# angela000/DQNFlappyBird

Hardware: AMD Instinct MI355X
Metric: env steps/sec (whole node) + DQN grad-steps/sec, 80x80x4 batch=32 (higher is better)
Workload: dtype f32

## Files before the change

### dqnflappybird_amd/csrc/fb_common.h

```cpp
#pragma once
#include <hip/hip_runtime.h>
#include <stdarg.h>
#include <stdint.h>
#include <stdio.h>
#include <string.h>
#include "../../include/fbdqn.h"

extern thread_local char fb_err_buf[512];
int fb_set_error(int code, const char *fmt, ...);

#define FB_CHECK_HIP(expr)                                                                     \
    do {                                                                                       \
        hipError_t e_ = (expr);                                                                \
        if (e_ != hipSuccess)                                                                  \
            return fb_set_error(FB_ERR_HIP, "%s failed: %s (%s:%d)", #expr, hipGetErrorString(e_), \
                                __FILE__, __LINE__);                                           \
    } while (0)

#define FB_REQUIRE(cond, ...)                                          \
    do {                                                               \
        if (!(cond)) return fb_set_error(FB_ERR_INVALID, __VA_ARGS__); \
    } while (0)

#define FB_LAUNCH_CHECK() FB_CHECK_HIP(hipGetLastError())
// ... 32 lines not shown
#define FB_STREAM_SAMPLE 2u
#define FB_STREAM_PER 3u
#define FB_STREAM_INIT 4u
#define FB_STREAM_EVAL 5u

struct fb_u4 { uint32_t x, y, z, w; };

__host__ __device__ static inline fb_u4 fb_philox(uint32_t k0, uint32_t k1, uint32_t c0, uint32_t c1,
                                                  uint32_t c2, uint32_t c3) {
#pragma unroll
    for (int r = 0; r < 10; r++) {
        uint64_t p0 = (uint64_t)0xD2511F53u * c0, p1 = (uint64_t)0xCD9E8D57u * c2;
        uint32_t n0 = (uint32_t)(p1 >> 32) ^ c1 ^ k0, n1 = (uint32_t)p1;
        uint32_t n2 = (uint32_t)(p0 >> 32) ^ c3 ^ k1, n3 = (uint32_t)p0;
        c0 = n0; c1 = n1; c2 = n2; c3 = n3;
        k0 += 0x9E3779B9u; k1 += 0xBB67AE85u;
    }
    return fb_u4{c0, c1, c2, c3};
}

struct FbMT { uint32_t mt[624]; uint32_t idx; };

struct FbSplitFlags;
struct FbSampleCtx { FbMT *mt; int *error; long long n; FbSplitFlags *gate; unsigned long long gate_val; long long newest_from; int wait_last_round; };
struct FbSampleRider { FbSampleCtx ctx; int k; long long setsize; long long *out; };
struct NetOff { int bf1, wv, bv, wq, bq, n; };
struct HeadCore {
    const float *hf; int stot, nks; float *q; int FC, A, dueling; NetOff off;
    uint8_t *actions; float epsilon; uint32_t seed_lo, seed_hi, step_lo, step_hi;
};
struct FbHeadRider { HeadCore c; const float *params; int on; unsigned long long *on_arrival; unsigned long long arrival_val; };
struct FbEvalRider {
    const int32_t *env_of;
    int32_t *ep_k, *ep_len;
    int32_t *score, *length; uint8_t *trunc;
    int episodes;
    unsigned *live;
    unsigned long long *done_step;
    unsigned long long step;
};
struct FbGatherCtx {
    long long cap; int n_envs, t_f, kind;
    const unsigned long long *bits; const uint8_t *act; const float *rew; const uint8_t *term; int *error;
    int nstep; double gamma;
};
struct FbGatherRider { FbGatherCtx c; long long steps; int B; const long long *idx; uint8_t *s, *s2, *a; float *r; uint8_t *t; };
int fb_replay_gather_rider(fb_replay_t h, int batch, const int64_t *idx, uint8_t *s, uint8_t *s2, uint8_t *a, float *r, uint8_t *t,
                           FbGatherRider *rider);
struct FbRingSrc { FbGatherCtx c; long long steps; const long long *idx; uint8_t *a; float *r; uint8_t *t; };
int fb_replay_ring_src(fb_replay_t h, int batch, const int64_t *idx, uint8_t *a, float *r, uint8_t *t, FbRingSrc *out);
int fb_qnet_train_step_ring(fb_qnet_t h, int algo, int batch, const FbRingSrc *ring, const float *isw, double gamma, float *loss,
                            float *abs_err, float *flat_grad, void *stream, const FbSampleRider *rider = nullptr, const struct FbSplitCtx *split = nullptr);
struct FbSplitFlags {
    unsigned long long c_entry, p0[7];
    unsigned long long trunk_done, p2[7];
    unsigned long long fc1_done, p3[7];
    unsigned long long env_done, p4[7];
    unsigned long long last_round, p8[7];
    unsigned clean_count;
    unsigned timeouts[7];
};
struct FbSplitCtx {
    hipStream_t tstream;
    FbSplitFlags *f;
    unsigned long long seq;
    const void *probed_stream; int probed_ok;
};
int fb_split_probe(FbSplitCtx *ctx, void *stream);
int fb_streams_concurrent(hipStream_t side, hipStream_t caller);
hipStream_t fb_side_stream_beside(hipStream_t caller, int priority, hipStream_t current, int *ok);
FbSplitCtx *fb_qnet_split_ctx(fb_qnet_t h);
int fb_replay_sample_gated(fb_replay_t h, int batch, int64_t *idx, const FbSplitCtx *ctx, void *stream, int wait_last_round = 0);
int fb_split_wait(const FbSplitCtx *ctx, const unsigned long long *flag, unsigned long long v, void *stream);
int fb_split_set(const FbSplitCtx *ctx, unsigned long long *flag, unsigned long long v, void *stream);
int fb_qnet_refresh_planes(fb_qnet_t h, void *stream);
int fb_qnet_profile_ring(fb_qnet_t h, int kernel, int reps, int algo, int batch, const FbRingSrc *ring, float *loss, void *stream);
struct FbPushRider { unsigned long long *bits; uint8_t *act; float *rew; uint8_t *term; long long *steps_dev; long long steps_new; };
int fb_env_step_rider(fb_env_t h, const uint8_t *actions, uint8_t *frames, uint64_t *frame_bits, float *reward, uint8_t *terminal,
                      int32_t *score, const FbSampleRider *rider, const FbPushRider *push, const FbHeadRider *head, void *stream);
int fb_qnet_num_actions(fb_qnet_t h);
int fb_qnet_is_c51(fb_qnet_t h);
int fb_qnet_c51_eval_head(fb_qnet_t h, const FbHeadRider *hd, int n, const int32_t *key_of, void *stream);
int fb_qnet_eval_trunk(fb_qnet_t h, const uint8_t *nib_states, int n, FbHeadRider *head, void *stream);
int fb_qnet_max_rows(fb_qnet_t h);
hipStream_t fb_qnet_side_stream(fb_qnet_t h);
void *fb_qnet_get_grad_event(fb_qnet_t h);
void *fb_qnet_take_grad_event_recorded(fb_qnet_t h);
int fb_qnet_check_step(fb_qnet_t h, int n_envs, int train_batch);
int fb_env_num_envs(fb_env_t h);
int fb_replay_num_envs(fb_replay_t h);
int fb_replay_is_prioritized(fb_replay_t h);
int fb_replay_check_gamma(fb_replay_t h, double gamma, const char *who);
int fb_replay_check_complete(fb_replay_t h, int pushes_ahead, const char *who);
double fb_replay_bootstrap_gamma(fb_replay_t h, double gamma);
int fb_replay_update_priorities_keep(fb_replay_t h, int batch, const int64_t *idx, const float *abs_err, void *stream);
// ... 16 lines not shown
```

### dqnflappybird_amd/csrc/fb_common.hip

```cpp
#include <execinfo.h>
#include <fcntl.h>
#include <signal.h>
#include <stdlib.h>
#include <unistd.h>
#include "fb_common.h"

thread_local char fb_err_buf[512] = "";

int fb_set_error(int code, const char *fmt, ...) {
    va_list ap;
    va_start(ap, fmt);
    vsnprintf(fb_err_buf, sizeof(fb_err_buf), fmt, ap);
    va_end(ap);
    return code;
}

extern "C" const char *fb_last_error(void) { return fb_err_buf; }

static struct sigaction fb_prev_abrt;
static bool fb_abrt_installed = false;
static int fb_abrt_log_fd = -1;
static void fb_abort_backtrace(int sig, siginfo_t *info, void *ctx) {
    static const char msg[] = "\n[libfbdqn] SIGABRT: native stack of the aborting thread\n";
    void *frames[64];
// ... 153 lines not shown
        if (hipStreamSynchronize(S) != hipSuccess || hipStreamSynchronize(C) != hipSuccess) return 0;
        unsigned long long st[3];
        if (hipMemcpy(st, &W->first, sizeof(st), hipMemcpyDeviceToHost) != hipSuccess) return 0;
        if (st[1] <= st[0]) return 0;
        const double frac = st[2] <= st[0] ? 0.0 : (double)(st[2] - st[0]) / (double)(st[1] - st[0]);
        if (frac < best) best = frac;
    }
    double worst_ratio = 1e9, alone_us = 0, beside_us = 0;
    for (int trial = 0; trial < 3 && worst_ratio >= 1.0; trial++) {
        unsigned long long st[5];
        const unsigned long long init[5] = {~0ull, 0ull, 0ull, ~0ull, 0ull};
        if (hipMemcpy(&W->first, init, sizeof(init), hipMemcpyHostToDevice) != hipSuccess) return 0;
        for (int i = 0; i < 8; i++) hipLaunchKernelGGL(probe_hold_kernel, dim3(1), dim3(64), 0, C, &W->first, &W->last, 50LL);
        if (hipStreamSynchronize(C) != hipSuccess || hipMemcpy(st, &W->first, sizeof(st), hipMemcpyDeviceToHost) != hipSuccess || st[1] <= st[0]) return 0;
        const double alone = (double)(st[1] - st[0]) / 100.0;
        if (hipMemcpy(&W->first, init, sizeof(init), hipMemcpyHostToDevice) != hipSuccess) return 0;
        hipLaunchKernelGGL(probe_hold_kernel, dim3(1), dim3(64), 0, S, &W->first2, &W->last2, 8000LL);
        for (int i = 0; i < 8; i++) hipLaunchKernelGGL(probe_hold_kernel, dim3(1), dim3(64), 0, C, &W->first, &W->last, 50LL);
        if (hipStreamSynchronize(S) != hipSuccess || hipStreamSynchronize(C) != hipSuccess) return 0;
        if (hipMemcpy(st, &W->first, sizeof(st), hipMemcpyDeviceToHost) != hipSuccess || st[1] <= st[0]) return 0;
        const double beside = (double)(st[1] - st[0]) / 100.0, ratio = beside / (2.0 * alone + 10.0);
        if (ratio < worst_ratio) { worst_ratio = ratio; alone_us = alone; beside_us = beside; }
    }
    if (getenv("FB_SIDE_PROBE_DEBUG"))
        fprintf(stderr, "[fb] side stream %p beside %p: a launch on it started %.2f of the way through a long launch on the caller's; eight small launches on the caller's took %.1f us beside "
                        "a long workgroup on it, %.1f alone\n", (void *)S, (void *)C, best, beside_us, alone_us);
    return best < 0.5 && worst_ratio < 1.0;
}

hipStream_t fb_side_stream_beside(hipStream_t C, int priority, hipStream_t current, int *ok) {
    bool good = current && fb_streams_concurrent(current, C);
    for (int attempt = 0; !good && attempt < 6; attempt++) {
        hipStream_t ts = nullptr;
        if (hipStreamCreateWithPriority(&ts, hipStreamNonBlocking, priority) != hipSuccess) break;
        if (current) { (void)hipStreamSynchronize(current); (void)hipStreamDestroy(current); }
        current = ts;
        good = fb_streams_concurrent(current, C);
    }
    (void)hipGetLastError();
    if (ok) *ok = good ? 1 : 0;
    return current;
}

static int fb_vec_split_flag = -1;
static bool fb_vec_split_enabled() {
    if (fb_vec_split_flag < 0) fb_vec_split_flag = !(getenv("FB_VEC_SPLIT") && atoi(getenv("FB_VEC_SPLIT")) == 0);
    return fb_vec_split_flag != 0;
}
extern "C" int fb_vec_step_set_schedule(int split) { fb_vec_split_flag = split ? 1 : 0; return FB_OK; }

// ... 8 lines not shown
        FB_REQUIRE(is_c51_algo(algo) == (fb_qnet_is_c51(net) != 0),
                   "%s: a C51 net takes a C51 algo (FB_ALGO_C51, _DOUBLE, _PER, _DOUBLE_PER), and those algos take a C51 net only (algo %d)", "fb_vec_step", algo);
        if (!is_per_algo(algo))
            FB_REQUIRE(!fb_replay_is_prioritized(replay), "%s: C51 trains from a uniform memory only (prioritized replay with C51 is not supported)", "fb_vec_step");
    }
    FB_REQUIRE(per == (fb_replay_is_prioritized(replay) != 0), "fb_vec_step: algo %d and the memory's kind (uniform / prioritized) do not match", algo);
    FB_REQUIRE(n_envs == fb_env_num_envs(env) && n_envs == fb_replay_num_envs(replay), "fb_vec_step: n_envs %d does not match the env (%d) / replay (%d) handles",
               n_envs, fb_env_num_envs(env), fb_replay_num_envs(replay));
    if (train) FB_REQUIRE(b->idx && b->s && b->s2 && b->a && b->r && b->t && b->loss, "fb_vec_step: NULL training buffer");
    {
        const int rc0 = fb_qnet_check_step(net, n_envs, train ? batch : -1);
        if (rc0 != FB_OK) return rc0;
        const int rc1 = fb_replay_check_gamma(replay, gamma, "fb_vec_step");
        if (rc1 != FB_OK) return rc1;
        const int rc2 = train ? fb_replay_check_complete(replay, 1, "fb_vec_step") : FB_OK;
        if (rc2 != FB_OK) return rc2;
    }
    gamma = fb_replay_bootstrap_gamma(replay, gamma);
    if (fb_vec_split_enabled() && train && !per && n_envs >= 256 && batch < 256 && fb_env_can_carry_head(env) && fb_qnet_num_actions(net) == 2 &&
        !fb_qnet_is_c51(net)) {
        hipStream_t A = fb_stream(stream);
        hipStreamCaptureStatus cap = hipStreamCaptureStatusNone;
        (void)hipStreamIsCapturing(A, &cap);
        FbSampleRider probe;
        FbSplitCtx *sc = cap == hipStreamCaptureStatusNone && fb_replay_sample_rider(replay, batch, b->idx, &probe) ? fb_qnet_split_ctx(net) : nullptr;
        if (sc && !fb_split_probe(sc, stream)) sc = nullptr;
        if (sc) {
            hipStream_t C = A, S = sc->tstream;
            FbSplitFlags *F = sc->f;
            sc->seq += 1;
            static const bool last_round_on = !(getenv("FB_SPLIT_LAST_ROUND") && atoi(getenv("FB_SPLIT_LAST_ROUND")) == 0);
            const int trunk_wgs = (n_envs + 4) / 5, wait_last_round = last_round_on && n_envs >= 4096 && trunk_wgs % 256 != 0;
            if (!fb_replay_sample_gated(replay, batch, b->idx, sc, C, wait_last_round)) { sc->seq -= 1; return fb_set_error(FB_ERR_HIP, "fb_vec_step: the gated draw could not be launched"); }
            int rc = fb_split_wait(sc, &F->c_entry, sc->seq, S);
            FbHeadRider hrider;
            if (rc == FB_OK) rc = fb_qnet_act_nib_rider(net, b->nib, n_envs, epsilon, seed, step, b->actions, &hrider, S, sc);
            if (rc != FB_OK) { (void)hipStreamSynchronize(S); return rc; }
            hrider.on_arrival = &F->fc1_done; hrider.arrival_val = sc->seq;
            FbPushRider prider;
            fb_replay_begin_push_rider(replay, &prider);
            FbRingSrc ring;
            rc = fb_replay_ring_src(replay, batch, b->idx, b->a, b->r, b->t, &ring);
            if (rc == FB_OK) rc = fb_qnet_train_step_ring(net, algo, batch, &ring, nullptr, gamma, b->loss, nullptr, b->flat_grad, C, nullptr, sc);
            const int rc2 = fb_env_step_rider(env, b->actions, nullptr, b->frame_bits, b->reward, b->terminal, b->score, nullptr, &prider, &hrider, S);
            const int rc3 = fb_split_set(sc, &F->env_done, sc->seq, S);
            return rc != FB_OK ? rc : rc2 != FB_OK ? rc2 : rc3;
        }
    }
    static const bool store_ahead = !(getenv("FB_PER_STORE_AHEAD") && atoi(getenv("FB_PER_STORE_AHEAD")) == 0);
    int sampled = 0;
    if (per && store_ahead && fb_replay_per_store_ahead(replay, stream) && train)
        sampled = fb_replay_sample_ahead(replay, batch, b->idx, b->isw, b->isw32, stream);
    FbHeadRider hrider;
    static const bool head_rides = !(getenv("FB_VEC_HEAD_RIDER") && atoi(getenv("FB_VEC_HEAD_RIDER")) == 0);
    const int have_h = head_rides && fb_env_can_carry_head(env) && fb_qnet_num_actions(net) == 2 && !fb_qnet_is_c51(net);
    int rc = have_h ? fb_qnet_act_nib_rider(net, b->nib, n_envs, epsilon, seed, step, b->actions, &hrider, stream)
                    : fb_qnet_act_nib(net, b->nib, n_envs, epsilon, seed, step, b->actions, nullptr, stream);
    if (rc != FB_OK) return rc;
    FbSampleRider srider;
    FbPushRider prider;
    static const bool sample_rides = !(getenv("FB_VEC_SAMPLE_RIDER") && atoi(getenv("FB_VEC_SAMPLE_RIDER")) == 0);
    const int have_s = train && sample_rides ? fb_replay_sample_rider(replay, batch, b->idx, &srider) : 0;
    const int have_p = fb_replay_begin_push_rider(replay, &prider);
    rc = fb_env_step_rider(env, b->actions, nullptr, b->frame_bits, b->reward, b->terminal, b->score, have_s ? &srider : nullptr,
                           have_p ? &prider : nullptr, have_h ? &hrider : nullptr, stream);
    if (rc != FB_OK) return rc;
// ... 74 lines not shown
```

### dqnflappybird_amd/csrc/fb_qnet.hip

```cpp
#include <math.h>
#include <stdlib.h>
#include "fb_common.h"

#ifndef FK_ABL
#define FK_ABL 0
#endif
#ifndef BW_ABL
#define BW_ABL 0
#endif

namespace {

typedef float f32x16 __attribute__((ext_vector_type(16)));

constexpr int OFF_W1 = 0, OFF_B1 = 8192, OFF_W2 = 8224, OFF_B2 = 40992, OFF_W3 = 41056, OFF_B3 = 77920,
              OFF_WF1 = 77984;
constexpr int CONV_PARAMS = OFF_WF1;
#include "fb_head.h"
#include "fb_sampler.h"
#include "fb_gather.h"
constexpr int MAXTB = 256;


struct Slice { const float *params; const uint8_t *states; int s_off, count; const uint16_t *w1s; int fshift; };
// ... 3080 lines not shown
    return FB_OK;
}

__global__ void flag_wait_kernel(const unsigned long long *flag, unsigned long long v, unsigned *timeouts) { if (threadIdx.x == 0) fb_flag_wait(flag, v, timeouts); }
__global__ void flag_set_kernel(unsigned long long *flag, unsigned long long v) { fb_flag_store(flag, v); }

FbSplitCtx *fb_qnet_split_ctx(fb_qnet_t h) {
    if (!h) return nullptr;
    if (h->split) return h->split->tstream ? h->split : nullptr;
    FbSplitCtx *c = new FbSplitCtx();
    memset(c, 0, sizeof(*c));
    h->split = c;
    int lo = 0, hi = 0;
    bool ok = hipMalloc((void **)&c->f, sizeof(FbSplitFlags)) == hipSuccess && hipMemset(c->f, 0, sizeof(FbSplitFlags)) == hipSuccess;
    hipStream_t ts = nullptr;
    ok = ok && hipDeviceGetStreamPriorityRange(&lo, &hi) == hipSuccess && hipStreamCreateWithPriority(&ts, hipStreamNonBlocking, lo) == hipSuccess;
    if (!ok) { (void)hipGetLastError(); return nullptr; }
    c->tstream = ts;
    return c;
}

int fb_split_probe(FbSplitCtx *c, void *stream) {
    if (!c || !c->tstream) return 0;
    if (c->probed_stream == stream && c->seq > 0) return c->probed_ok;
    int lo = 0, hi = 0, ok = 0;
    if (hipDeviceGetStreamPriorityRange(&lo, &hi) != hipSuccess) return 0;
    c->tstream = fb_side_stream_beside(reinterpret_cast<hipStream_t>(stream), lo, c->tstream, &ok);
    c->probed_stream = stream; c->probed_ok = ok;
    return ok;
}

int fb_split_wait(const FbSplitCtx *c, const unsigned long long *flag, unsigned long long v, void *stream) {
    hipLaunchKernelGGL(flag_wait_kernel, dim3(1), dim3(64), 0, fb_stream(stream), flag, v, &c->f->timeouts[1]);
    FB_LAUNCH_CHECK();
    return FB_OK;
}

int fb_split_set(const FbSplitCtx *, unsigned long long *flag, unsigned long long v, void *stream) {
    hipLaunchKernelGGL(flag_set_kernel, dim3(1), dim3(1), 0, fb_stream(stream), flag, v);
    FB_LAUNCH_CHECK();
    return FB_OK;
}

extern "C" int fb_qnet_split_stats(fb_qnet_t h, int64_t *steps_host, int64_t *clean_host) {
    FB_REQUIRE(h && steps_host && clean_host, "fb_qnet_split_stats: NULL argument");
    *steps_host = 0; *clean_host = 0;
    if (!h->split || !h->split->tstream) return FB_OK;
    FB_CHECK_HIP(hipDeviceSynchronize());
    unsigned v[8] = {0};
    FB_CHECK_HIP(hipMemcpy(v, &h->split->f->clean_count, sizeof(v), hipMemcpyDeviceToHost));
    FB_REQUIRE(!(v[1] | v[2] | v[3] | v[4] | v[5] | v[6]), "fb_qnet_split_stats: waits between the two chains of the split schedule gave up after 1 s (the draw %u, the side stream's entry %u, "
// ... 729 lines not shown
```

### dqnflappybird_amd/csrc/fb_replay.hip

```cpp
#include <math.h>
#include "fb_common.h"

namespace {

constexpr int WORDS = 100;
constexpr int MAXB = 256;
constexpr int MAXH = 23;

struct ReplayDev {
    long long steps;
    long long per_pointer, per_size;
    double beta;
    unsigned int done_ctr;
    unsigned int philox_calls;
    int error;
};

struct ReplayParams {
    long long cap;
    int n_envs, t_f, kind;
    unsigned long long *bits;
    uint8_t *act; float *rew; uint8_t *term;
    ReplayDev *dev;
    double *tree, *maxt, *mint;
// ... 65 lines not shown
template <bool CURRENT>
__global__ __launch_bounds__(256) void gather_kernel(ReplayParams P, long long steps, int B, const long long *__restrict__ idx,
                                                     uint4 *__restrict__ s, uint4 *__restrict__ s2,
                                                     uint8_t *__restrict__ a, float *__restrict__ r,
                                                     uint8_t *__restrict__ t) {
    gather_body<CURRENT>(gather_ctx(P), steps, B, idx, s, s2, a, r, t, (long long)blockIdx.x * 256 + threadIdx.x);
}

__device__ __forceinline__ FbSampleCtx sample_ctx(const ReplayParams &P, long long steps) {
    return FbSampleCtx{P.mt, &P.dev->error, population(P, steps)};
}

__global__ __launch_bounds__(64) void sample_cpython_kernel(ReplayParams P, int k, long long setsize,
                                                            long long *__restrict__ out) {
    __shared__ uint32_t mt[624];
    __shared__ int pool[FB_SAMPLE_POOL + FB_SAMPLE_TAB];
    sample_cpython_body(sample_ctx(P, P.dev->steps), k, setsize, out, mt, pool);
}

__global__ __launch_bounds__(64) void sample_gated_kernel(FbSampleRider r) {
    __shared__ uint32_t mt[624];
    __shared__ int pool[FB_SAMPLE_POOL + FB_SAMPLE_TAB];
    sample_cpython_body(r.ctx, r.k, r.setsize, r.out, mt, pool);
}

__global__ __launch_bounds__(64) void push_sample_kernel(ReplayParams P, long long steps, const uint8_t *__restrict__ frames,
                                                         const unsigned long long *__restrict__ fbits,
                                                         const uint8_t *__restrict__ a, const float *__restrict__ r,
                                                         const uint8_t *__restrict__ t, int k, long long setsize,
                                                         long long *__restrict__ out) {
    __shared__ uint32_t mt[624];
    __shared__ int pool[FB_SAMPLE_POOL + FB_SAMPLE_TAB];
    if (blockIdx.x == gridDim.x - 1) { sample_cpython_body(sample_ctx(P, steps + 1), k, setsize, out, mt, pool); return; }
    const int lane = threadIdx.x;
    for (int e = blockIdx.x; e < P.n_envs; e += gridDim.x - 1) {
        unsigned long long *dst = P.bits + frame_off(P, steps + 1, e);
        if (fbits) {
            for (int w = lane; w < WORDS; w += 64) dst[w] = fbits[(size_t)e * WORDS + w];
        } else {
            for (int w = 0; w < WORDS; w++) {
                const unsigned long long m = __ballot(frames[(size_t)e * 6400 + w * 64 + lane] != 0);
                if (lane == 0) dst[w] = m;
            }
        }
        if (lane == 0) {
            const size_t mo = (size_t)(steps % P.t_f) * P.n_envs + e;
// ... 462 lines not shown
        for (;;) {
            const long long cl = 2 * parent + 1;
            if (cl >= len) break;
            const double left = P.tree[cl];
            if (v <= left) parent = cl;
            else { v -= left; parent = cl + 1; }
        }
        const double prob = P.tree[parent] / total;
        const double min_prob = P.mint[0] / total;
        idx_out[tid] = parent;
        const double wgt = pow(prob / min_prob, -beta);
        isw_out[tid] = wgt;
        if (isw32_out) isw32_out[tid] = (float)wgt;
    }
    if (tid == 0) { P.dev->beta = beta; P.dev->philox_calls = call + 1; }
}

}

struct fb_replay {
    ReplayParams P;
    FbMT *h_mt;
    long long host_steps;
    int per_mode;
    hipStream_t side;
    hipEvent_t ev_fork, ev_store, ev_upd;
    bool store_ahead;
    bool upd_pending;
    bool store_forked;
    const void *side_for; bool side_checked; int side_ok; int side_prio;
};

static bool per_side_usable(fb_replay *h, void *stream) {
    if (!h->side) return false;
    if (h->side_checked && h->side_for == stream) return h->side_ok != 0;
    if (h->store_ahead || h->upd_pending) return h->side_checked && h->side_ok != 0;
    h->side = fb_side_stream_beside(fb_stream(stream), h->side_prio, h->side, &h->side_ok);
    h->side_for = stream; h->side_checked = true;
    return h->side_ok != 0;
}


static int per_join(fb_replay *h, hipStream_t st) {
    if (h->upd_pending) {
        FB_CHECK_HIP(hipStreamWaitEvent(st, h->ev_upd, 0));
        h->upd_pending = false;
    }
    return FB_OK;
}

static int replay_create(int64_t capacity, int n_envs, int kind, int ring_n, fb_replay_t *out) {
    fb_replay *h = new fb_replay();
    memset(h, 0, sizeof(*h));
    ReplayParams &P = h->P;
    P.cap = capacity; P.n_envs = n_envs; P.kind = kind;
    P.nstep = 1; P.gamma = 0.0;
    P.t_f = (int)((capacity + n_envs - 1) / n_envs) + ring_n + 5;
    const size_t slots = (size_t)P.t_f * n_envs;
    hipError_t e = hipMalloc(&P.bits, slots * WORDS * sizeof(unsigned long long));
    if (e == hipSuccess) e = hipMemset(P.bits, 0, slots * WORDS * sizeof(unsigned long long));
    if (e == hipSuccess) e = hipMalloc(&P.act, slots);
    if (e == hipSuccess) e = hipMemset(P.act, 0, slots);
    if (e == hipSuccess) e = hipMalloc(&P.rew, slots * sizeof(float));
    if (e == hipSuccess) e = hipMemset(P.rew, 0, slots * sizeof(float));
    if (e == hipSuccess) e = hipMalloc(&P.term, slots);
    if (e == hipSuccess) e = hipMemset(P.term, 0, slots);
    if (e == hipSuccess) e = hipMalloc(&P.dev, sizeof(ReplayDev));
    if (e == hipSuccess) e = hipMemset(P.dev, 0, sizeof(ReplayDev));
    if (e == hipSuccess) e = hipMalloc(&P.mt, sizeof(FbMT));
    if (e == hipSuccess && kind == FB_REPLAY_PER) {
        const size_t nb = sizeof(double) * (size_t)(2 * capacity - 1);
        e = hipMalloc(&P.tree, nb);
        if (e == hipSuccess) e = hipMalloc(&P.maxt, nb);
        if (e == hipSuccess) e = hipMalloc(&P.mint, nb);
    }
    if (e != hipSuccess) {
        fb_set_error(e == hipErrorOutOfMemory ? FB_ERR_NOMEM : FB_ERR_HIP, "fb_replay_create: %s", hipGetErrorString(e));
        fb_replay_destroy(h);
        return e == hipErrorOutOfMemory ? FB_ERR_NOMEM : FB_ERR_HIP;
    }
    if (kind == FB_REPLAY_PER) {
        int prio_lo = 0, prio_hi = 0;
        (void)hipDeviceGetStreamPriorityRange(&prio_lo, &prio_hi);
        h->side_prio = prio_hi;
        if (hipStreamCreateWithPriority(&h->side, hipStreamNonBlocking, h->side_prio) != hipSuccess ||
            hipEventCreateWithFlags(&h->ev_fork, hipEventDisableTiming) != hipSuccess ||
            hipEventCreateWithFlags(&h->ev_store, hipEventDisableTiming) != hipSuccess ||
            hipEventCreateWithFlags(&h->ev_upd, hipEventDisableTiming) != hipSuccess) {
            fb_set_error(FB_ERR_HIP, "fb_replay_create: stream / event creation failed");
            fb_replay_destroy(h);
            return FB_ERR_HIP;
        }
// ... 10 lines not shown
    FB_REQUIRE(n_envs >= 1 && n_envs <= (1 << 22), "fb_replay_create: n_envs out of range");
    FB_REQUIRE(kind == FB_REPLAY_UNIFORM || kind == FB_REPLAY_PER, "fb_replay_create: kind must be 0 or 1");
    return replay_create(capacity, n_envs, kind, 1, out);
}

extern "C" int fb_replay_create_nstep(int64_t capacity, int n_envs, int kind, int n, double gamma, fb_replay_t *out) {
    FB_REQUIRE(out, "fb_replay_create_nstep: out is NULL");
    FB_REQUIRE(capacity >= 1 && capacity < (1ll << 22), "fb_replay_create_nstep: capacity %lld out of range", (long long)capacity);
    FB_REQUIRE(n_envs >= 1 && n_envs <= (1 << 22), "fb_replay_create_nstep: n_envs out of range");
    FB_REQUIRE(kind == FB_REPLAY_UNIFORM || kind == FB_REPLAY_PER, "fb_replay_create_nstep: kind must be 0 or 1");
    FB_REQUIRE(n >= 1 && n <= FB_NSTEP_MAX, "fb_replay_create_nstep: n = %d is outside 1..%d", n, FB_NSTEP_MAX);
    FB_REQUIRE(capacity >= (long long)n * n_envs, "fb_replay_create_nstep: capacity %lld < n x n_envs = %lld", (long long)capacity,
               (long long)n * n_envs);
    const int rc = replay_create(capacity, n_envs, kind, kind == FB_REPLAY_PER ? n : 1, out);
    if (rc != FB_OK) return rc;
    (*out)->P.nstep = n;
    (*out)->P.gamma = n > 1 ? gamma : 0.0;
    return FB_OK;
}

extern "C" int fb_replay_destroy(fb_replay_t h) {
    if (!h) return FB_OK;
    ReplayParams &P = h->P;
    void *ptrs[] = {P.bits, P.act, P.rew, P.term, P.dev, P.mt, P.tree, P.maxt, P.mint};
    for (void *p : ptrs) if (p) (void)hipFree(p);
    if (h->side) { (void)hipStreamSynchronize(h->side); (void)hipStreamDestroy(h->side); }
    if (h->ev_fork) (void)hipEventDestroy(h->ev_fork);
    if (h->ev_store) (void)hipEventDestroy(h->ev_store);
    if (h->ev_upd) (void)hipEventDestroy(h->ev_upd);
    delete h;
    return FB_OK;
}

extern "C" int fb_replay_seed(fb_replay_t h, int rng_kind, uint64_t seed) {
    FB_REQUIRE(h, "fb_replay_seed: NULL handle");
    FB_REQUIRE(rng_kind >= 0 && rng_kind <= 2, "fb_replay_seed: rng_kind must be 0 (cpython), 1 (philox) or 2 (numpy)");
    FbMT s;
    if (rng_kind == FB_RNG_NUMPY) fb_mt_init_genrand_host(&s, (uint32_t)seed);
    else {
        uint32_t key[2] = {(uint32_t)seed, (uint32_t)(seed >> 32)};
        fb_mt_init_by_array_host(&s, key, key[1] ? 2 : 1);
    }
    FB_CHECK_HIP(hipDeviceSynchronize());
    FB_CHECK_HIP(hipMemcpy(h->P.mt, &s, sizeof(FbMT), hipMemcpyHostToDevice));
    h->P.rng_kind = rng_kind;
    h->P.seed_lo = (uint32_t)seed; h->P.seed_hi = (uint32_t)(seed >> 32);
    return FB_OK;
}

extern "C" int fb_replay_reset(fb_replay_t h, const uint8_t *frames, const uint64_t *frame_bits, void *stream) {
    FB_REQUIRE(h, "fb_replay_reset: NULL handle");
    h->host_steps = 0;
    ReplayParams &P = h->P;
    hipStream_t st = fb_stream(stream);
    if (P.kind == FB_REPLAY_PER) {
        if (h->side) {
            FB_CHECK_HIP(hipStreamSynchronize(h->side));
            h->store_ahead = false; h->upd_pending = false;
        }
        const long long nn = 2 * P.cap - 1;
        FB_CHECK_HIP(hipMemsetAsync(P.tree, 0, sizeof(double) * nn, st));
        FB_CHECK_HIP(hipMemsetAsync(P.maxt, 0, sizeof(double) * nn, st));
        hipLaunchKernelGGL(fill_f64_kernel, dim3(256), dim3(256), 0, st, P.mint, nn, (double)INFINITY);
        FB_LAUNCH_CHECK();
    }
    if (!frames && !frame_bits) {
        FB_CHECK_HIP(hipMemsetAsync(P.bits, 0, (size_t)P.n_envs * WORDS * sizeof(unsigned long long), st));
        FB_CHECK_HIP(hipMemsetAsync(P.dev, 0, sizeof(ReplayDev), st));
        ReplayDev d; memset(&d, 0, sizeof(d)); d.beta = 0.4;
        FB_CHECK_HIP(hipStreamSynchronize(st));
        FB_CHECK_HIP(hipMemcpy(P.dev, &d, sizeof(d), hipMemcpyHostToDevice));
        return FB_OK;
    }
    hipLaunchKernelGGL(reset_kernel, dim3(P.n_envs), dim3(64), 0, st, P, frames, (const unsigned long long *)frame_bits);
    FB_LAUNCH_CHECK();
    return FB_OK;
}

extern "C" int fb_replay_push(fb_replay_t h, const uint8_t *frames, const uint64_t *frame_bits, const uint8_t *actions,
                              const float *rewards, const uint8_t *terminals, void *stream) {
    FB_REQUIRE(h && actions && rewards && terminals, "fb_replay_push: NULL argument");
    FB_REQUIRE((frames != nullptr) != (frame_bits != nullptr), "fb_replay_push: give exactly one of frames / frame_bits");
    ReplayParams &P = h->P;
    hipStream_t st = fb_stream(stream);
    hipLaunchKernelGGL(push_kernel, dim3(P.n_envs < 512 ? P.n_envs : 512), dim3(64), 0, st, P, h->host_steps, frames, (const unsigned long long *)frame_bits,
                       actions, rewards, terminals);
    FB_LAUNCH_CHECK();
    h->host_steps += 1;
    return fb_replay_finish_push(h, stream);
}

int fb_replay_finish_push(fb_replay_t h, void *stream) {
    ReplayParams &P = h->P;
    hipStream_t st = fb_stream(stream);
    if (P.kind == FB_REPLAY_PER) {
        if (h->store_ahead) {
            h->store_ahead = false;
            h->upd_pending = false;
            FB_CHECK_HIP(hipStreamWaitEvent(st, h->ev_store, 0));
            return FB_OK;
        }
        if (h->host_steps < P.nstep) return FB_OK;
        const int rcj = per_join(h, st);
        if (rcj != FB_OK) return rcj;
        if (h->per_mode == FB_PER_FAST) hipLaunchKernelGGL(per_store_fast_kernel, dim3(1), dim3(1024), 0, st, P, P.n_envs);
        else hipLaunchKernelGGL(per_store_kernel, dim3(1), dim3(1024), 0, st, P, P.n_envs);
        FB_LAUNCH_CHECK();
    }
    return FB_OK;
}

// ... 25 lines not shown

static long long cpython_setsize(int batch) {
    long long setsize = 21;
    if (batch > 5) setsize += (long long)pow(4.0, ceil(log((double)batch * 3.0) / log(4.0)));
    return setsize;
}

extern "C" int fb_replay_push_sample(fb_replay_t h, const uint8_t *frames, const uint64_t *frame_bits, const uint8_t *actions,
                                     const float *rewards, const uint8_t *terminals, int batch, int64_t *idx, void *stream) {
    FB_REQUIRE(h && actions && rewards && terminals && idx, "fb_replay_push_sample: NULL argument");
    FB_REQUIRE((frames != nullptr) != (frame_bits != nullptr), "fb_replay_push_sample: give exactly one of frames / frame_bits");
    FB_REQUIRE(batch >= 1 && batch <= MAXB, "fb_replay_push_sample: batch must be in 1..%d", MAXB);
    ReplayParams &P = h->P;
    if (P.kind != FB_REPLAY_UNIFORM || P.rng_kind != FB_RNG_CPYTHON) {
        int rc = fb_replay_push(h, frames, frame_bits, actions, rewards, terminals, stream);
        if (rc != FB_OK) return rc;
        return fb_replay_sample(h, batch, nullptr, idx, nullptr, stream);
    }
    hipLaunchKernelGGL(push_sample_kernel, dim3((P.n_envs < 512 ? P.n_envs : 512) + 1), dim3(64), 0, fb_stream(stream), P, h->host_steps,
                       frames, (const unsigned long long *)frame_bits, actions, rewards, terminals, batch, cpython_setsize(batch),
                       (long long *)idx);
    FB_LAUNCH_CHECK();
    h->host_steps += 1;
    return FB_OK;
}

int fb_replay_num_envs(fb_replay_t h) { return h ? h->P.n_envs : 0; }

extern "C" int fb_replay_set_n_step(fb_replay_t h, int n, double gamma) {
    FB_REQUIRE(h, "fb_replay_set_n_step: NULL handle");
    FB_REQUIRE(h->P.kind == FB_REPLAY_UNIFORM, "fb_replay_set_n_step: a prioritized memory's n is fixed when it is created: use fb_replay_create_nstep");
    FB_REQUIRE(n >= 1 && n <= FB_NSTEP_MAX, "fb_replay_set_n_step: n = %d is outside 1..%d", n, FB_NSTEP_MAX);
    FB_REQUIRE(h->P.cap >= (long long)n * h->P.n_envs, "fb_replay_set_n_step: capacity %lld < n x n_envs = %lld", (long long)h->P.cap,
               (long long)n * h->P.n_envs);
    h->P.nstep = n;
    h->P.gamma = n > 1 ? gamma : 0.0;
    return FB_OK;
}

extern "C" int fb_replay_get_n_step(fb_replay_t h, int *n_host, double *gamma_host) {
    FB_REQUIRE(h && n_host && gamma_host, "fb_replay_get_n_step: NULL argument");
    *n_host = h->P.nstep; *gamma_host = h->P.gamma;
    return FB_OK;
}

int fb_replay_check_gamma(fb_replay_t h, double gamma, const char *who) {
    FB_REQUIRE(h->P.nstep == 1 || gamma == h->P.gamma, "%s: gamma %.17g differs from the gamma %.17g of the memory's %d-step view", who, gamma,
               h->P.gamma, h->P.nstep);
    return FB_OK;
}

int fb_replay_check_complete(fb_replay_t h, int pushes_ahead, const char *who) {
    if (h->P.kind != FB_REPLAY_PER || h->host_steps + pushes_ahead >= h->P.nstep) return FB_OK;
    return fb_set_error(FB_ERR_STATE, "%s: the %d-step prioritized memory holds no complete transition before %d pushes since its reset (%lld)", who,
                        h->P.nstep, h->P.nstep, h->host_steps + pushes_ahead);
}

double fb_replay_bootstrap_gamma(fb_replay_t h, double gamma) {
    if (h->P.nstep == 1) return gamma;
    double g = 1.0;
    for (int k = 0; k < h->P.nstep; k++) g *= h->P.gamma;
    return g;
}

int fb_replay_is_prioritized(fb_replay_t h) { return h && h->P.kind == FB_REPLAY_PER; }

int fb_replay_begin_push_rider(fb_replay_t h, FbPushRider *push) {
    ReplayParams &P = h->P;
    const long long steps = h->host_steps;
    push->bits = P.bits + (size_t)((steps + 1) % P.t_f) * P.n_envs * WORDS;
    const size_t mo = (size_t)(steps % P.t_f) * P.n_envs;
    push->act = P.act + mo; push->rew = P.rew + mo; push->term = P.term + mo;
    push->steps_dev = &P.dev->steps; push->steps_new = steps + 1;
    h->host_steps += 1;
    return 1;
}

int fb_replay_gather_rider(fb_replay_t h, int batch, const int64_t *idx, uint8_t *s, uint8_t *s2, uint8_t *a, float *r, uint8_t *t,
                           FbGatherRider *rider) {
    if (!h || !idx || !s || !s2 || !a || !r || !t || batch < 1) return 0;
    rider->c = gather_ctx(h->P); rider->steps = h->host_steps; rider->B = batch; rider->idx = (const long long *)idx;
    rider->s = s; rider->s2 = s2; rider->a = a; rider->r = r; rider->t = t;
    return 1;
}

int fb_replay_sample_rider(fb_replay_t h, int batch, int64_t *idx, FbSampleRider *rider, int pushes_ahead) {
    const ReplayParams &P = h->P;
    if (P.kind != FB_REPLAY_UNIFORM || P.rng_kind != FB_RNG_CPYTHON || batch < 1 || batch > MAXB || !idx) return 0;
    rider->ctx = FbSampleCtx{P.mt, &P.dev->error, population(P, h->host_steps + pushes_ahead)};
    rider->k = batch; rider->setsize = cpython_setsize(batch); rider->out = (long long *)idx;
    return 1;
}

int fb_replay_sample_gated(fb_replay_t h, int batch, int64_t *idx, const FbSplitCtx *ctx, void *stream, int wait_last_round) {
    FbSampleRider r;
    if (!h || !ctx || !fb_replay_sample_rider(h, batch, idx, &r, 1)) return 0;
    r.ctx.gate = ctx->f; r.ctx.gate_val = ctx->seq; r.ctx.wait_last_round = wait_last_round;
    r.ctx.newest_from = r.ctx.n - h->P.n_envs;
    hipLaunchKernelGGL(sample_gated_kernel, dim3(1), dim3(64), 0, fb_stream(stream), r);
    return hipGetLastError() == hipSuccess;
}

extern "C" int fb_replay_current_state(fb_replay_t h, uint8_t *states, void *stream) {
    FB_REQUIRE(h && states, "fb_replay_current_state: NULL argument");
    ReplayParams &P = h->P;
    const long long threads = (long long)P.n_envs * 1600;
    hipLaunchKernelGGL(gather_kernel<true>, dim3((unsigned)((threads + 255) / 256)), dim3(256), 0, fb_stream(stream), P,
                       h->host_steps, P.n_envs, (const long long *)nullptr, (uint4 *)states, (uint4 *)nullptr, (uint8_t *)nullptr,
                       (float *)nullptr, (uint8_t *)nullptr);
    FB_LAUNCH_CHECK();
    return FB_OK;
}

extern "C" int fb_replay_sample(fb_replay_t h, int batch, const double *uniforms, int64_t *idx, double *isw, void *stream) {
    return fb_replay_sample_f32(h, batch, uniforms, idx, isw, nullptr, stream);
}

int fb_replay_sample_f32(fb_replay_t h, int batch, const double *uniforms, int64_t *idx, double *isw, float *isw32, void *stream) {
    FB_REQUIRE(h && idx, "fb_replay_sample: NULL argument");
    FB_REQUIRE(batch >= 1 && batch <= MAXB, "fb_replay_sample: batch must be in 1..%d", MAXB);
    ReplayParams &P = h->P;
    hipStream_t st = fb_stream(stream);
    if (P.kind == FB_REPLAY_PER) {
        FB_REQUIRE(isw, "fb_replay_sample: PER needs isw");
        const int rcc = fb_replay_check_complete(h, 0, "fb_replay_sample");
        if (rcc != FB_OK) return rcc;
        const int rcj = per_join(h, st);
        if (rcj != FB_OK) return rcj;
        hipLaunchKernelGGL(per_sample_kernel, dim3(1), dim3(256), 0, st, P, batch, uniforms, (long long *)idx, isw, isw32);
    } else if (P.rng_kind == FB_RNG_PHILOX) {
        hipLaunchKernelGGL(sample_philox_kernel, dim3(1), dim3(256), 0, st, P, batch, (long long *)idx);
    } else {
        hipLaunchKernelGGL(sample_cpython_kernel, dim3(1), dim3(64), 0, st, P, batch, cpython_setsize(batch), (long long *)idx);
    }
    FB_LAUNCH_CHECK();
    return FB_OK;
}

int fb_replay_ring_src(fb_replay_t h, int batch, const int64_t *idx, uint8_t *a, float *r, uint8_t *t, FbRingSrc *out) {
    FB_REQUIRE(h && idx && a && r && t && out, "fb_replay_ring_src: NULL argument");
    FB_REQUIRE(batch >= 1 && batch <= MAXB, "fb_replay_ring_src: batch out of range");
    *out = FbRingSrc{gather_ctx(h->P), h->host_steps, (const long long *)idx, a, r, t};
    return FB_OK;
}

// ... 177 lines not shown
extern "C" int fb_replay_load_state(fb_replay_t h, const void *blob_host, size_t bytes) {
    FB_REQUIRE(h && blob_host && bytes >= sizeof(ReplayBlobHeader), "fb_replay_load_state: bad argument");
    ReplayBlobHeader hd;
    memcpy(&hd, blob_host, sizeof(hd));
    size_t need = 0;
    fb_replay_state_bytes(h, &need);
    FB_REQUIRE(hd.magic == REPLAY_BLOB_MAGIC && hd.version == 1, "fb_replay_load_state: not a replay checkpoint");
    FB_REQUIRE(hd.cap == h->P.cap && hd.n_envs == h->P.n_envs && hd.kind == h->P.kind,
               "fb_replay_load_state: the checkpoint is of a memory with capacity %lld, %d envs, kind %d; this one has %lld, %d, %d",
               (long long)hd.cap, hd.n_envs, hd.kind, (long long)h->P.cap, h->P.n_envs, h->P.kind);
    const int t_f1 = (int)((h->P.cap + h->P.n_envs - 1) / h->P.n_envs) + 6;
    FB_REQUIRE(hd.t_f == h->P.t_f, "fb_replay_load_state: the checkpoint is of a prioritized memory with n = %d (a ring of %d time slots); this one has "
               "n = %d (%d)", hd.t_f - t_f1 + 1, hd.t_f, h->P.t_f - t_f1 + 1, h->P.t_f);
    FB_REQUIRE(hd.total_bytes == need && bytes >= need, "fb_replay_load_state: the checkpoint holds %llu bytes, this memory's state is %zu (%zu given)",
               (unsigned long long)hd.total_bytes, need, bytes);
    FB_CHECK_HIP(hipDeviceSynchronize());
    BlobPart parts[9];
    const int n = blob_parts(h, parts);
    const char *o = (const char *)blob_host + sizeof(hd);
    for (int i = 0; i < n; i++) {
        FB_CHECK_HIP(hipMemcpy(parts[i].dev, o, parts[i].bytes, hipMemcpyHostToDevice));
        o += (parts[i].bytes + 15) & ~(size_t)15;
    }
    h->host_steps = hd.host_steps; h->P.rng_kind = hd.rng_kind; h->per_mode = hd.per_mode; h->P.seed_lo = hd.seed_lo; h->P.seed_hi = hd.seed_hi;
    return FB_OK;
}
```

### dqnflappybird_amd/csrc/fb_sampler.h

```cpp
#pragma once

constexpr int FB_SAMPLE_MAXB = 256;
constexpr int FB_SAMPLE_POOL = 1100, FB_SAMPLE_TAB = 1024;
constexpr int FB_SAMPLE_LDS_WORDS = 624 + FB_SAMPLE_POOL + FB_SAMPLE_TAB;

__device__ __forceinline__ uint32_t mt_temper(uint32_t y) {
    y ^= (y >> 11); y ^= (y << 7) & 0x9d2c5680u; y ^= (y << 15) & 0xefc60000u; y ^= (y >> 18);
    return y;
}

__device__ __forceinline__ void mt_regen(uint32_t *mt, int lane) {
    for (int base = 0; base < 624; base += 64) {
        const int i = base + lane;
        uint32_t v = 0;
        if (i < 624) {
            const uint32_t y = (mt[i] & 0x80000000u) | (mt[i == 623 ? 0 : i + 1] & 0x7fffffffu);
            v = mt[i + 397 < 624 ? i + 397 : i + 397 - 624] ^ (y >> 1) ^ ((y & 1u) ? 0x9908b0dfu : 0u);
        }
        __builtin_amdgcn_wave_barrier();
        if (i < 624) mt[i] = v;
        __builtin_amdgcn_wave_barrier();
    }
}

__device__ __forceinline__ void set_sel(long long (&sel)[4], int i, int lane, long long v) {
#pragma unroll
    for (int q = 0; q < 4; q++) if (q == (i >> 6) && lane == (i & 63)) sel[q] = v;
}

__device__ __forceinline__ void sample_cpython_body(const FbSampleCtx &P, int k, long long setsize,
                                                    long long *__restrict__ out, uint32_t *mt, int *pool) {
    const int lane = threadIdx.x;
    if (P.gate && lane == 0) fb_flag_store(&P.gate->c_entry, P.gate_val);
    for (int i = lane; i < 624; i += 64) mt[i] = P.mt->mt[i];
    uint32_t idx = P.mt->idx;
    bool regenerated = false;
    const long long n = P.n;
    if (k > n || k > FB_SAMPLE_MAXB) {
        if (lane == 0) *P.error = 2;
        for (int i = lane; i < k; i += 64) out[i] = 0;
        return;
    }
    __builtin_amdgcn_wave_barrier();
    long long sel[4] = {-1, -1, -1, -1};
    if (n > setsize) {
        const int shift = __builtin_clz((uint32_t)n);
        int i = 0;
        if (k <= 64) {
            if (idx >= 624) { mt_regen(mt, lane); idx = 0; regenerated = true; }
            const int avail = 624 - (int)idx, take = avail < 64 ? avail : 64;
// ... 70 lines not shown
#pragma unroll
            for (int q = 0; q < 4; q++) sel[q] = q * 64 + lane < k ? (long long)(uint32_t)pool[q * 64 + lane] : -1;
        }
    } else {
        for (int i = lane; i < (int)n; i += 64) pool[i] = i;
        __builtin_amdgcn_wave_barrier();
        for (int i = 0; i < k; i++) {
            const uint32_t m = (uint32_t)(n - i);
            const int nbits = 32 - __builtin_clz(m);
            uint32_t r;
            do {
                if (idx >= 624) { mt_regen(mt, lane); idx = 0; regenerated = true; }
                r = mt_temper(mt[idx++]) >> (32 - nbits);
            } while (r >= m);
            const long long res = pool[r];
            __builtin_amdgcn_wave_barrier();
            if (lane == 0) pool[r] = pool[m - 1];
            __builtin_amdgcn_wave_barrier();
            set_sel(sel, i, lane, res);
        }
    }
#pragma unroll
    for (int q = 0; q < 4; q++) if (q * 64 + lane < k) out[q * 64 + lane] = sel[q];
    if (regenerated) for (int i = lane; i < 624; i += 64) P.mt->mt[i] = mt[i];
    if (lane == 0) P.mt->idx = idx;
    if (P.gate) {
        bool dirty = false;
#pragma unroll
        for (int q = 0; q < 4; q++) dirty |= q * 64 + lane < k && sel[q] >= P.newest_from;
        dirty = __any(dirty);
        if (lane == 0) {
            if (!dirty) atomicAdd(&P.gate->clean_count, 1u);
            fb_flag_wait(&P.gate->env_done, dirty ? P.gate_val : P.gate_val - 1, &P.gate->timeouts[0]);
            if (P.wait_last_round) fb_flag_wait(&P.gate->last_round, P.gate_val, &P.gate->timeouts[5]);
        }
    }
}
```

Baseline: 11.27 million.

## Pre-draw next replay batch inside the train step, adopt it at next split head

The next step's CPython-compatible replay sample is now drawn during the current train step, which already carries a sample rider. The draw writes to a shadow Mersenne Twister state and a pre-draw buffer. On the next split step, if an epoch counter shows no intervening RNG or replay mutation, a tiny head kernel copies the pre-drawn indices and performs the gate wait, then the MT state buffers are swapped. This takes the serial MT sampling off the critical head of the train chain. The cost is extra bookkeeping, and any missed epoch bump could break RNG equivalence.

```diff
diff --git a/dqnflappybird_amd/csrc/fb_common.h b/dqnflappybird_amd/csrc/fb_common.h
--- a/dqnflappybird_amd/csrc/fb_common.h
+++ b/dqnflappybird_amd/csrc/fb_common.h
@@ -78,7 +78,8 @@
 struct FbMT { uint32_t mt[624]; uint32_t idx; };
 
 struct FbSplitFlags;
-struct FbSampleCtx { FbMT *mt; int *error; long long n; FbSplitFlags *gate; unsigned long long gate_val; long long newest_from; int wait_last_round; };
+struct FbSampleCtx { FbMT *mt; int *error; long long n; FbSplitFlags *gate; unsigned long long gate_val; long long newest_from; int wait_last_round;
+                     FbMT *mt_out; int *dirty_out; };
 struct FbSampleRider { FbSampleCtx ctx; int k; long long setsize; long long *out; };
 struct NetOff { int bf1, wv, bv, wq, bq, n; };
 struct HeadCore {
@@ -120,13 +121,16 @@
     hipStream_t tstream;
     FbSplitFlags *f;
     unsigned long long seq;
-    const void *probed_stream; int probed_ok;
+    const void *probed_stream; int probed, probed_ok;
 };
 int fb_split_probe(FbSplitCtx *ctx, void *stream);
 int fb_streams_concurrent(hipStream_t side, hipStream_t caller);
 hipStream_t fb_side_stream_beside(hipStream_t caller, int priority, hipStream_t current, int *ok);
 FbSplitCtx *fb_qnet_split_ctx(fb_qnet_t h);
 int fb_replay_sample_gated(fb_replay_t h, int batch, int64_t *idx, const FbSplitCtx *ctx, void *stream, int wait_last_round = 0);
+int fb_replay_draws_cpython(fb_replay_t h, int batch);
+int fb_replay_predraw_rider(fb_replay_t h, int batch, void *stream, FbSampleRider *rider);
+void fb_replay_predraw_cancel(fb_replay_t h);
 int fb_split_wait(const FbSplitCtx *ctx, const unsigned long long *flag, unsigned long long v, void *stream);
 int fb_split_set(const FbSplitCtx *ctx, unsigned long long *flag, unsigned long long v, void *stream);
 int fb_qnet_refresh_planes(fb_qnet_t h, void *stream);
diff --git a/dqnflappybird_amd/csrc/fb_common.hip b/dqnflappybird_amd/csrc/fb_common.hip
--- a/dqnflappybird_amd/csrc/fb_common.hip
+++ b/dqnflappybird_amd/csrc/fb_common.hip
@@ -199,10 +199,11 @@
         const double beside = (double)(st[1] - st[0]) / 100.0, ratio = beside / (2.0 * alone + 10.0);
         if (ratio < worst_ratio) { worst_ratio = ratio; alone_us = alone; beside_us = beside; }
     }
+    const bool forced_fail = getenv("FB_SIDE_PROBE_FAIL") && atoi(getenv("FB_SIDE_PROBE_FAIL")) == 1;
     if (getenv("FB_SIDE_PROBE_DEBUG"))
         fprintf(stderr, "[fb] side stream %p beside %p: a launch on it started %.2f of the way through a long launch on the caller's; eight small launches on the caller's took %.1f us beside "
-                        "a long workgroup on it, %.1f alone\n", (void *)S, (void *)C, best, beside_us, alone_us);
-    return best < 0.5 && worst_ratio < 1.0;
+                        "a long workgroup on it, %.1f alone%s\n", (void *)S, (void *)C, best, beside_us, alone_us, forced_fail ? " (forced to fail)" : "");
+    return best < 0.5 && worst_ratio < 1.0 && !forced_fail;
 }
 
 hipStream_t fb_side_stream_beside(hipStream_t C, int priority, hipStream_t current, int *ok) {
@@ -257,8 +258,7 @@
         hipStream_t A = fb_stream(stream);
         hipStreamCaptureStatus cap = hipStreamCaptureStatusNone;
         (void)hipStreamIsCapturing(A, &cap);
-        FbSampleRider probe;
-        FbSplitCtx *sc = cap == hipStreamCaptureStatusNone && fb_replay_sample_rider(replay, batch, b->idx, &probe) ? fb_qnet_split_ctx(net) : nullptr;
+        FbSplitCtx *sc = cap == hipStreamCaptureStatusNone && fb_replay_draws_cpython(replay, batch) ? fb_qnet_split_ctx(net) : nullptr;
         if (sc && !fb_split_probe(sc, stream)) sc = nullptr;
         if (sc) {
             hipStream_t C = A, S = sc->tstream;
@@ -266,7 +266,7 @@
             sc->seq += 1;
             static const bool last_round_on = !(getenv("FB_SPLIT_LAST_ROUND") && atoi(getenv("FB_SPLIT_LAST_ROUND")) == 0);
             const int trunk_wgs = (n_envs + 4) / 5, wait_last_round = last_round_on && n_envs >= 4096 && trunk_wgs % 256 != 0;
-            if (!fb_replay_sample_gated(replay, batch, b->idx, sc, C, wait_last_round)) { sc->seq -= 1; return fb_set_error(FB_ERR_HIP, "fb_vec_step: the gated draw could not be launched"); }
+            if (!fb_replay_sample_gated(replay, batch, b->idx, sc, C, wait_last_round)) { sc->seq -= 1; return fb_set_error(FB_ERR_HIP, "fb_vec_step: the head of the train chain could not be launched"); }
             int rc = fb_split_wait(sc, &F->c_entry, sc->seq, S);
             FbHeadRider hrider;
             if (rc == FB_OK) rc = fb_qnet_act_nib_rider(net, b->nib, n_envs, epsilon, seed, step, b->actions, &hrider, S, sc);
@@ -276,7 +276,11 @@
             fb_replay_begin_push_rider(replay, &prider);
             FbRingSrc ring;
             rc = fb_replay_ring_src(replay, batch, b->idx, b->a, b->r, b->t, &ring);
-            if (rc == FB_OK) rc = fb_qnet_train_step_ring(net, algo, batch, &ring, nullptr, gamma, b->loss, nullptr, b->flat_grad, C, nullptr, sc);
+            static const bool predraw_on = !(getenv("FB_SPLIT_PREDRAW") && atoi(getenv("FB_SPLIT_PREDRAW")) == 0);
+            FbSampleRider pre;
+            const int pre_on = rc == FB_OK && predraw_on && fb_replay_predraw_rider(replay, batch, stream, &pre);
+            if (rc == FB_OK) rc = fb_qnet_train_step_ring(net, algo, batch, &ring, nullptr, gamma, b->loss, nullptr, b->flat_grad, C, pre_on ? &pre : nullptr, sc);
+            if (pre_on && rc != FB_OK) fb_replay_predraw_cancel(replay);
             const int rc2 = fb_env_step_rider(env, b->actions, nullptr, b->frame_bits, b->reward, b->terminal, b->score, nullptr, &prider, &hrider, S);
             const int rc3 = fb_split_set(sc, &F->env_done, sc->seq, S);
             return rc != FB_OK ? rc : rc2 != FB_OK ? rc2 : rc3;
diff --git a/dqnflappybird_amd/csrc/fb_qnet.hip b/dqnflappybird_amd/csrc/fb_qnet.hip
--- a/dqnflappybird_amd/csrc/fb_qnet.hip
+++ b/dqnflappybird_amd/csrc/fb_qnet.hip
@@ -3126,11 +3126,11 @@
 
 int fb_split_probe(FbSplitCtx *c, void *stream) {
     if (!c || !c->tstream) return 0;
-    if (c->probed_stream == stream && c->seq > 0) return c->probed_ok;
+    if (c->probed && c->probed_stream == stream) return c->probed_ok;
     int lo = 0, hi = 0, ok = 0;
     if (hipDeviceGetStreamPriorityRange(&lo, &hi) != hipSuccess) return 0;
     c->tstream = fb_side_stream_beside(reinterpret_cast<hipStream_t>(stream), lo, c->tstream, &ok);
-    c->probed_stream = stream; c->probed_ok = ok;
+    c->probed_stream = stream; c->probed = 1; c->probed_ok = ok;
     return ok;
 }
 
diff --git a/dqnflappybird_amd/csrc/fb_replay.hip b/dqnflappybird_amd/csrc/fb_replay.hip
--- a/dqnflappybird_amd/csrc/fb_replay.hip
+++ b/dqnflappybird_amd/csrc/fb_replay.hip
@@ -111,6 +111,16 @@
     __shared__ uint32_t mt[624];
     __shared__ int pool[FB_SAMPLE_POOL + FB_SAMPLE_TAB];
     sample_cpython_body(r.ctx, r.k, r.setsize, r.out, mt, pool);
+}
+
+struct PreDraw { long long idx[MAXB]; int dirty; int pad; };
+
+__global__ __launch_bounds__(64) void split_head_kernel(FbSampleCtx g, const PreDraw *__restrict__ pre, int k, long long *__restrict__ out) {
+    const int lane = threadIdx.x;
+    if (lane == 0) fb_flag_store(&g.gate->c_entry, g.gate_val);
+    for (int i = lane; i < k; i += 64) out[i] = pre->idx[i];
+    const bool dirty = pre->dirty != 0;
+    if (lane == 0) split_gate_wait(g, dirty);
 }
 
 __global__ __launch_bounds__(64) void push_sample_kernel(ReplayParams P, long long steps, const uint8_t *__restrict__ frames,
@@ -619,6 +629,10 @@
     ReplayParams P;
     FbMT *h_mt;
     long long host_steps;
+    FbMT *mt_shadow;
+    PreDraw *pre;
+    unsigned long long epoch;
+    struct { bool pending; unsigned long long epoch; int batch; long long n; const void *stream; } pd;
     int per_mode;
     hipStream_t side;
     hipEvent_t ev_fork, ev_store, ev_upd;
@@ -665,6 +679,8 @@
     if (e == hipSuccess) e = hipMalloc(&P.dev, sizeof(ReplayDev));
     if (e == hipSuccess) e = hipMemset(P.dev, 0, sizeof(ReplayDev));
     if (e == hipSuccess) e = hipMalloc(&P.mt, sizeof(FbMT));
+    if (e == hipSuccess && kind == FB_REPLAY_UNIFORM) e = hipMalloc(&h->mt_shadow, sizeof(FbMT));
+    if (e == hipSuccess && kind == FB_REPLAY_UNIFORM) e = hipMalloc(&h->pre, sizeof(PreDraw));
     if (e == hipSuccess && kind == FB_REPLAY_PER) {
         const size_t nb = sizeof(double) * (size_t)(2 * capacity - 1);
         e = hipMalloc(&P.tree, nb);
@@ -721,7 +737,7 @@
 extern "C" int fb_replay_destroy(fb_replay_t h) {
     if (!h) return FB_OK;
     ReplayParams &P = h->P;
-    void *ptrs[] = {P.bits, P.act, P.rew, P.term, P.dev, P.mt, P.tree, P.maxt, P.mint};
+    void *ptrs[] = {P.bits, P.act, P.rew, P.term, P.dev, P.mt, P.tree, P.maxt, P.mint, h->mt_shadow, h->pre};
     for (void *p : ptrs) if (p) (void)hipFree(p);
     if (h->side) { (void)hipStreamSynchronize(h->side); (void)hipStreamDestroy(h->side); }
     if (h->ev_fork) (void)hipEventDestroy(h->ev_fork);
@@ -744,12 +760,14 @@
     FB_CHECK_HIP(hipMemcpy(h->P.mt, &s, sizeof(FbMT), hipMemcpyHostToDevice));
     h->P.rng_kind = rng_kind;
     h->P.seed_lo = (uint32_t)seed; h->P.seed_hi = (uint32_t)(seed >> 32);
+    h->epoch += 1;
     return FB_OK;
 }
 
 extern "C" int fb_replay_reset(fb_replay_t h, const uint8_t *frames, const uint64_t *frame_bits, void *stream) {
     FB_REQUIRE(h, "fb_replay_reset: NULL handle");
     h->host_steps = 0;
+    h->epoch += 1;
     ReplayParams &P = h->P;
     hipStream_t st = fb_stream(stream);
     if (P.kind == FB_REPLAY_PER) {
@@ -786,6 +804,7 @@
                        actions, rewards, terminals);
     FB_LAUNCH_CHECK();
     h->host_steps += 1;
+    h->epoch += 1;
     return fb_replay_finish_push(h, stream);
 }
 
@@ -857,6 +876,7 @@
                        (long long *)idx);
     FB_LAUNCH_CHECK();
     h->host_steps += 1;
+    h->epoch += 1;
     return FB_OK;
 }
 
@@ -870,6 +890,7 @@
                (long long)n * h->P.n_envs);
     h->P.nstep = n;
     h->P.gamma = n > 1 ? gamma : 0.0;
+    h->epoch += 1;
     return FB_OK;
 }
 
@@ -908,6 +929,7 @@
     push->act = P.act + mo; push->rew = P.rew + mo; push->term = P.term + mo;
     push->steps_dev = &P.dev->steps; push->steps_new = steps + 1;
     h->host_steps += 1;
+    h->epoch += 1;
     return 1;
 }
 
@@ -919,17 +941,49 @@
     return 1;
 }
 
+int fb_replay_draws_cpython(fb_replay_t h, int batch) {
+    return h && h->P.kind == FB_REPLAY_UNIFORM && h->P.rng_kind == FB_RNG_CPYTHON && batch >= 1 && batch <= MAXB;
+}
+
 int fb_replay_sample_rider(fb_replay_t h, int batch, int64_t *idx, FbSampleRider *rider, int pushes_ahead) {
     const ReplayParams &P = h->P;
-    if (P.kind != FB_REPLAY_UNIFORM || P.rng_kind != FB_RNG_CPYTHON || batch < 1 || batch > MAXB || !idx) return 0;
+    if (!fb_replay_draws_cpython(h, batch) || !idx) return 0;
     rider->ctx = FbSampleCtx{P.mt, &P.dev->error, population(P, h->host_steps + pushes_ahead)};
     rider->k = batch; rider->setsize = cpython_setsize(batch); rider->out = (long long *)idx;
+    h->epoch += 1;
     return 1;
 }
 
+int fb_replay_predraw_rider(fb_replay_t h, int batch, void *stream, FbSampleRider *rider) {
+    h->pd.pending = false;
+    if (!fb_replay_draws_cpython(h, batch) || !h->mt_shadow || !h->pre) return 0;
+    const ReplayParams &P = h->P;
+    const long long n = population(P, h->host_steps + 1);
+    if (batch > n) return 0;
+    rider->ctx = FbSampleCtx{P.mt, &P.dev->error, n, nullptr, 0, n - P.n_envs, 0, h->mt_shadow, &h->pre->dirty};
+    rider->k = batch; rider->setsize = cpython_setsize(batch); rider->out = h->pre->idx;
+    h->pd.pending = true; h->pd.epoch = h->epoch; h->pd.batch = batch; h->pd.n = n; h->pd.stream = stream;
+    return 1;
+}
+
+void fb_replay_predraw_cancel(fb_replay_t h) { if (h) h->pd.pending = false; }
+
 int fb_replay_sample_gated(fb_replay_t h, int batch, int64_t *idx, const FbSplitCtx *ctx, void *stream, int wait_last_round) {
+    if (!h || !ctx || !fb_replay_draws_cpython(h, batch) || !idx) return 0;
+    const long long n = population(h->P, h->host_steps + 1);
+    const bool adopt = h->pd.pending && h->pd.epoch == h->epoch && h->pd.batch == batch && h->pd.n == n && h->pd.stream == stream;
+    h->pd.pending = false;
+    if (adopt) {
+        FbSampleCtx g{};
+        g.gate = ctx->f; g.gate_val = ctx->seq; g.wait_last_round = wait_last_round;
+        hipLaunchKernelGGL(split_head_kernel, dim3(1), dim3(64), 0, fb_stream(stream), g, (const PreDraw *)h->pre, batch, (long long *)idx);
+        if (hipGetLastError() != hipSuccess) return 0;
+        FbMT *t = h->P.mt; h->P.mt = h->mt_shadow; h->mt_shadow = t;
+        h->epoch += 1;
+        return 1;
+    }
     FbSampleRider r;
-    if (!h || !ctx || !fb_replay_sample_rider(h, batch, idx, &r, 1)) return 0;
+    fb_replay_sample_rider(h, batch, idx, &r, 1);
     r.ctx.gate = ctx->f; r.ctx.gate_val = ctx->seq; r.ctx.wait_last_round = wait_last_round;
     r.ctx.newest_from = r.ctx.n - h->P.n_envs;
     hipLaunchKernelGGL(sample_gated_kernel, dim3(1), dim3(64), 0, fb_stream(stream), r);
@@ -956,6 +1010,7 @@
     FB_REQUIRE(batch >= 1 && batch <= MAXB, "fb_replay_sample: batch must be in 1..%d", MAXB);
     ReplayParams &P = h->P;
     hipStream_t st = fb_stream(stream);
+    h->epoch += 1;
     if (P.kind == FB_REPLAY_PER) {
         FB_REQUIRE(isw, "fb_replay_sample: PER needs isw");
         const int rcc = fb_replay_check_complete(h, 0, "fb_replay_sample");
@@ -1179,6 +1234,7 @@
         FB_CHECK_HIP(hipMemcpy(parts[i].dev, o, parts[i].bytes, hipMemcpyHostToDevice));
         o += (parts[i].bytes + 15) & ~(size_t)15;
     }
+    h->epoch += 1;
     h->host_steps = hd.host_steps; h->P.rng_kind = hd.rng_kind; h->per_mode = hd.per_mode; h->P.seed_lo = hd.seed_lo; h->P.seed_hi = hd.seed_hi;
     return FB_OK;
 }
diff --git a/dqnflappybird_amd/csrc/fb_sampler.h b/dqnflappybird_amd/csrc/fb_sampler.h
--- a/dqnflappybird_amd/csrc/fb_sampler.h
+++ b/dqnflappybird_amd/csrc/fb_sampler.h
@@ -26,6 +26,12 @@
 __device__ __forceinline__ void set_sel(long long (&sel)[4], int i, int lane, long long v) {
 #pragma unroll
     for (int q = 0; q < 4; q++) if (q == (i >> 6) && lane == (i & 63)) sel[q] = v;
+}
+
+__device__ __forceinline__ void split_gate_wait(const FbSampleCtx &P, bool dirty) {
+    if (!dirty) atomicAdd(&P.gate->clean_count, 1u);
+    fb_flag_wait(&P.gate->env_done, dirty ? P.gate_val : P.gate_val - 1, &P.gate->timeouts[0]);
+    if (P.wait_last_round) fb_flag_wait(&P.gate->last_round, P.gate_val, &P.gate->timeouts[5]);
 }
 
 __device__ __forceinline__ void sample_cpython_body(const FbSampleCtx &P, int k, long long setsize,
@@ -142,17 +148,15 @@
     }
 #pragma unroll
     for (int q = 0; q < 4; q++) if (q * 64 + lane < k) out[q * 64 + lane] = sel[q];
-    if (regenerated) for (int i = lane; i < 624; i += 64) P.mt->mt[i] = mt[i];
-    if (lane == 0) P.mt->idx = idx;
-    if (P.gate) {
+    FbMT *mo = P.mt_out ? P.mt_out : P.mt;
+    if (regenerated || mo != P.mt) for (int i = lane; i < 624; i += 64) mo->mt[i] = mt[i];
+    if (lane == 0) mo->idx = idx;
+    if (P.gate || P.dirty_out) {
         bool dirty = false;
 #pragma unroll
         for (int q = 0; q < 4; q++) dirty |= q * 64 + lane < k && sel[q] >= P.newest_from;
         dirty = __any(dirty);
-        if (lane == 0) {
-            if (!dirty) atomicAdd(&P.gate->clean_count, 1u);
-            fb_flag_wait(&P.gate->env_done, dirty ? P.gate_val : P.gate_val - 1, &P.gate->timeouts[0]);
-            if (P.wait_last_round) fb_flag_wait(&P.gate->last_round, P.gate_val, &P.gate->timeouts[5]);
-        }
+        if (P.dirty_out && lane == 0) *P.dirty_out = dirty ? 1 : 0;
+        if (P.gate && lane == 0) split_gate_wait(P, dirty);
     }
 }
```

Result: no change. 11.29 million, median of 6 (+0.2%).
